# JNP-Solutions/Slacken

Hardware: AMD Instinct MI355X
Metric: classify_throughput_150bp_standard224scale (higher is better)
Workload: dtype u64

## Files before the change

slacken_amd/csrc/lane.hip:

```cpp
#include "engine.h"

#include <algorithm>
#include <cstddef>
#include <cstdio>
#include <cstdlib>

namespace slk {

#ifndef SLK_LANE_LW
#define SLK_LANE_LW 4
#endif
constexpr int LW = SLK_LANE_LW;
constexpr int QCAP = 128;
#ifndef SLK_SBLK
#define SLK_SBLK 5
#endif
constexpr int SBLK = SLK_SBLK;
#ifndef SLK_OMAP
#define SLK_OMAP 12
#endif
constexpr int OMAP = SLK_OMAP;
constexpr int OMAP_CNT_BITS = 10;
constexpr uint32_t OMAP_CNT_MASK = (1u << OMAP_CNT_BITS) - 1;

struct __attribute__((aligned(16))) LaneLds {
  uint64_t q_key[QCAP];
  uint32_t q_meta[QCAP];
  uint64_t stash[128];
  uint32_t found[64];
  uint4 sbuf[(SBLK - 1) * 64];
  uint32_t omap[OMAP * 64];
  uint32_t o_flags[64];
  uint64_t rb[64];
  uint16_t q_ord[QCAP];
};

#ifdef SLK_TUNING
#define SLK_TUNE(...) __VA_ARGS__
#define SLK_TUNE_ON(bit) ((dbg & (bit)) != 0)
#else
#define SLK_TUNE(...)
#define SLK_TUNE_ON(bit) false
#endif

#ifndef SLK_PROBE_NT
#define SLK_PROBE_NT 0
#endif
__device__ __forceinline__ ulonglong2 SLK_PROBE_LOAD(const ulonglong2 *p) {
#if SLK_PROBE_NT
  ulonglong2 v;
  v.x = __builtin_nontemporal_load(&p->x);
  v.y = __builtin_nontemporal_load(&p->y);
  return v;
#else
  return *p;
#endif
}

__device__ __forceinline__ void lane_wave_sync() {
  __builtin_amdgcn_fence(__ATOMIC_RELEASE, "wavefront");
  __builtin_amdgcn_wave_barrier();
  __builtin_amdgcn_fence(__ATOMIC_ACQUIRE, "wavefront");
}
__device__ __forceinline__ uint64_t lmin64(uint64_t a, uint64_t b) { return a < b ? a : b; }

template <bool LONG>
__device__ __forceinline__ void fold_hit(LaneLds *L, uint32_t *ocnt, bool in, uint32_t meta, int32_t taxon) {
  if (in && taxon != 0) {
    const int owner = meta & 63;
    const int32_t kmers = (int32_t)((meta >> 7) & 0x1FFF);
    if (meta & 64) atomicAdd(&L->o_flags[owner], 1u);
    uint32_t slot = (uint32_t)(((uint64_t)((uint32_t)taxon * 0x9E3779B1u) * (uint32_t)OMAP) >> 32);
    int p = 0;
    if (LONG) {
      for (; p < OMAP; p++) {
        uint32_t old = atomicCAS(&L->omap[slot * 64 + owner], 0u, (uint32_t)taxon);
        if (old == 0u || old == (uint32_t)taxon) { atomicAdd(&ocnt[slot * 64 + owner], (uint32_t)kmers); break; }
        slot = (slot + 1 == (uint32_t)OMAP) ? 0u : slot + 1;
      }
    } else {
      const uint32_t fresh = ((uint32_t)taxon << OMAP_CNT_BITS) | (uint32_t)kmers;
      for (; p < OMAP; p++) {
        uint32_t old = atomicCAS(&L->omap[slot * 64 + owner], 0u, fresh);
        if (old == 0u) break;
        if ((old >> OMAP_CNT_BITS) == (uint32_t)taxon) { atomicAdd(&L->omap[slot * 64 + owner], (uint32_t)kmers); break; }
        slot = (slot + 1 == (uint32_t)OMAP) ? 0u : slot + 1;
      }
    }
    if (p == OMAP) atomicOr(&L->o_flags[owner], 0x80000000u);
  }
}

constexpr int PG = 64 / LPB;
template <bool HITS, bool LONG>
__device__ __forceinline__ int probe_batch(LaneLds *L, uint32_t *ocnt, const TableView &T, int qhead, int qn, int cnt, int lane, int dbg,
                                           int32_t *hit_meta, int32_t *hit_taxon) {
  const uint64_t NO_TAG = ~0ULL;
  const bool in = lane < cnt;
  const int qi = (qhead + lane) & (QCAP - 1);
  const uint64_t key = L->q_key[qi];
  const uint32_t meta = L->q_meta[qi];
  const uint32_t ord = HITS ? L->q_ord[qi] : 0u;
  const uint64_t h = fmix64(key);
  uint32_t home;
  uint64_t rem_hi;
  table_slot(T.g, h, home, rem_hi);
  uint4 st;
  const uint32_t disp = (meta >> 20) & 255;
  st.x = table_bucket(T.g, home, disp);
  st.y = 0;
  const uint64_t tag = in ? (rem_hi + disp) : NO_TAG;
  st.z = (uint32_t)tag; st.w = (uint32_t)(tag >> 32);
  ((uint4 *)L->stash)[lane] = st;
  L->found[lane] = 0;
  lane_wave_sync();
  const int g = lane / LPB, c = lane % LPB;
  const uint64_t tmask = (1ULL << T.g.taxon_bits) - 1;
  const char *cellbase = (const char *)T.cells + c * 16;
  ulonglong2 cell[LPB];
#pragma unroll
  for (int s = 0; s < LPB; s++) {
    uint32_t bkt = ((const uint4 *)L->stash)[s * PG + g].x;
    SLK_TUNE(if (dbg & 4) bkt &= 1023u;)
    cell[s] = SLK_PROBE_LOAD((const ulonglong2 *)(cellbase + ((uint64_t)bkt << BUCKET_SHIFT)));
  }
  constexpr uint64_t GROUP_LSB = LPB == 4 ? 0x1111111111111111ULL : 0x0101010101010101ULL;
  int requeued = 0;
#pragma unroll
  for (int s = 0; s < LPB; s++) {
    const uint2 tg = *(const uint2 *)&((const uint4 *)L->stash)[s * PG + g].z;
    const uint64_t want = ((uint64_t)tg.y << 32) | tg.x;
    const bool act = want != NO_TAG;
    const bool e0 = cell[s].x == 0, e1 = cell[s].y == 0;
    const bool m0 = act && !e0 && cell_tag(T.g, cell[s].x) == want;
    const bool m1 = act && !e1 && cell_tag(T.g, cell[s].y) == want;
    if (m0 || m1) L->found[s * PG + g] = (uint32_t)((m0 ? cell[s].x : cell[s].y) & tmask);
    const bool closed = T.g.flag != 0 && c == 0 && (cell[s].x & T.g.flag) == 0;
    const uint64_t B = __ballot(m0 || m1 || e0 || e1 || !act || closed);
    uint64_t any = B;
#pragma unroll
    for (int i = 1; i < LPB; i <<= 1) any |= any >> i;
    if ((any & GROUP_LSB) != GROUP_LSB) {
      const int qj = (qhead + s * PG + g) & (QCAP - 1);
      const uint32_t m_old = L->q_meta[qj];
      const bool again = c == 0 && ((B >> (g * LPB)) & ((1u << LPB) - 1)) == 0 && (int)((m_old >> 20) & 255) < T.max_disp;
      const uint64_t k_old = L->q_key[qj];
      const uint16_t o_old = HITS ? L->q_ord[qj] : (uint16_t)0;
      const uint64_t R = __ballot(again);
      lane_wave_sync();
      if (again) {
        const int slot = (qhead + qn + requeued + __builtin_amdgcn_mbcnt_hi((uint32_t)(R >> 32), __builtin_amdgcn_mbcnt_lo((uint32_t)R, 0))) & (QCAP - 1);
        L->q_key[slot] = k_old;
        L->q_meta[slot] = m_old + (1u << 20);
        if (HITS) L->q_ord[slot] = o_old;
      }
      requeued += __popcll(R);
    }
  }
  lane_wave_sync();
  const int32_t taxon = (int32_t)L->found[lane];
  if (!SLK_TUNE_ON(2)) fold_hit<LONG>(L, ocnt, in, meta, taxon);
  if (HITS && in) {
    const uint64_t at = L->rb[meta & 63] + ord;
    hit_taxon[at] = ext_taxon(T, taxon);
    hit_meta[at] = pack_meta((int32_t)((meta >> 7) & 0x1FFF), 1, (meta >> 6) & 1);
  }
  lane_wave_sync();
  return requeued;
}

#ifndef SLK_STREAM_NT
#define SLK_STREAM_NT 0
#endif
#ifndef SLK_APPLY_ROWS
#define SLK_APPLY_ROWS 4
#endif
template <class T> __device__ __forceinline__ T SLK_STREAM_LOAD(const T *p) {
#if SLK_STREAM_NT
  return __builtin_nontemporal_load(p);
#else
  return *p;
#endif
}
template <class T> __device__ __forceinline__ void SLK_STREAM_STORE(T *p, T v) {
#if SLK_STREAM_NT
  __builtin_nontemporal_store(v, p);
#else
  *p = v;
#endif
}

__device__ __forceinline__ uint64_t lane_readlane64(uint64_t v, int src) {
  uint32_t lo = __builtin_amdgcn_readlane((uint32_t)v, src), hi = __builtin_amdgcn_readlane((uint32_t)(v >> 32), src);
  return ((uint64_t)hi << 32) | lo;
}
__device__ __forceinline__ uint32_t shard_owner(uint64_t key, uint32_t ns) {
  const uint64_t h = fmix64(key);
  return (ns & (ns - 1)) == 0 ? (uint32_t)(h & (ns - 1)) : (uint32_t)(h % ns);
}
__device__ __forceinline__ uint64_t side_load(const ShardIO &S, uint64_t batch, int lane) {
  const uint64_t i = batch * 64 + (uint64_t)lane;
  return i < S.side_n ? (uint64_t)SLK_STREAM_LOAD(&S.side_keys[i]) : 0;
}
__device__ __forceinline__ void side_probe(LaneLds *L, const TableView &T, const ShardIO &S, int lane, uint64_t batch, uint64_t key, int dbg) {
  const uint64_t base = batch * 64;
  if (base >= S.side_n) return;
  const uint64_t i = base + (uint64_t)lane;
  const bool in = i < S.side_n;
  const uint64_t h = fmix64(key);
  uint32_t home;
  uint64_t rem_hi;
  table_slot(T.g, h, home, rem_hi);
  const uint64_t tag = in ? rem_hi : ~0ULL;
  uint4 st;
  st.x = home; st.y = 0; st.z = (uint32_t)tag; st.w = (uint32_t)(tag >> 32);
  ((uint4 *)L->stash)[lane] = st;
  L->found[lane] = 0;
  lane_wave_sync();
  const int g = lane / LPB, c = lane % LPB;
  const uint64_t tmask = (1ULL << T.g.taxon_bits) - 1;
  const char *cellbase = (const char *)T.cells + c * 16;
  ulonglong2 cell[LPB];
#pragma unroll
  for (int s = 0; s < LPB; s++) {
    uint32_t bkt = ((const uint4 *)L->stash)[s * PG + g].x;
    SLK_TUNE(if (dbg & 4) bkt &= 1023u;)
    cell[s] = SLK_PROBE_LOAD((const ulonglong2 *)(cellbase + ((uint64_t)bkt << BUCKET_SHIFT)));
  }
  uint32_t unresolved = 0;
#pragma unroll
  for (int s = 0; s < LPB; s++) {
    const uint2 tg = *(const uint2 *)&((const uint4 *)L->stash)[s * PG + g].z;
    const uint64_t want = ((uint64_t)tg.y << 32) | tg.x;
    const bool act = want != ~0ULL;
    const bool e0 = cell[s].x == 0, e1 = cell[s].y == 0;
    const bool m0 = act && !e0 && cell_tag(T.g, cell[s].x) == want;
    const bool m1 = act && !e1 && cell_tag(T.g, cell[s].y) == want;
    if (m0 || m1) L->found[s * PG + g] = (uint32_t)((m0 ? cell[s].x : cell[s].y) & tmask);
    const bool closed = T.g.flag != 0 && c == 0 && (cell[s].x & T.g.flag) == 0;
    const uint64_t B = __ballot(m0 || m1 || e0 || e1 || !act || closed);
    if (((B >> (g * LPB)) & ((1u << LPB) - 1)) == 0) unresolved |= 1u << s;
  }
  lane_wave_sync();
  int32_t taxon = (int32_t)L->found[lane];
  const uint32_t ur = (uint32_t)__shfl((int)unresolved, (lane % PG) * LPB);
  if (in && ((ur >> (lane / PG)) & 1)) {
    for (int d = 1; d <= T.max_disp; d++) {
      const ulonglong2 *b = (const ulonglong2 *)(T.cells + ((uint64_t)table_bucket(T.g, home, (uint32_t)d) * CELLS));
      const uint64_t want = rem_hi | (uint64_t)d;
      bool has_empty = false, closed = false;
      int32_t hit = 0;
#pragma unroll
      for (int q = 0; q < LPB; q++) {
        const ulonglong2 v = b[q];
        has_empty |= (v.x == 0) | (v.y == 0);
        if (q == 0) closed = T.g.flag != 0 && (v.x & T.g.flag) == 0;
        if (v.x != 0 && cell_tag(T.g, v.x) == want) hit = (int32_t)(v.x & tmask);
        if (v.y != 0 && cell_tag(T.g, v.y) == want) hit = (int32_t)(v.y & tmask);
      }
      if (hit) { taxon = hit; break; }
      if (has_empty || closed) break;
    }
  }
  if (in && !SLK_TUNE_ON(128)) SLK_STREAM_STORE(&S.side_out[i], ext_taxon(T, taxon));
  lane_wave_sync();
}

template <bool HITS>
__device__ __forceinline__ void apply_rows(LaneLds *L, const ApplyJob &J, int lane, uint64_t row0, uint32_t nrows) {
  const uint32_t ns = (uint32_t)J.n_shards;
  constexpr int U = SLK_APPLY_ROWS;
  for (uint32_t b = 0; b < nrows; b += U) {
    uint64_t at[U];
    bool in[U];
#pragma unroll
    for (int u = 0; u < U; u++) {
      in[u] = false;
      at[u] = 0;
      if (b + u < nrows) {
        uint32_t off = 0;
        for (uint32_t sh = 0; sh < ns; sh++) {
          const uint4 e = J.batch_log[(row0 + b + u) * ns + sh];
          const uint32_t cnt = e.z;
          if (cnt == 0) continue;
          if ((uint32_t)lane >= off && (uint32_t)lane < off + cnt) {
            in[u] = true;
            const uint32_t i = (uint32_t)lane - off;
            at[u] = (uint64_t)sh * J.cap + (i < e.w ? e.x + i : e.y + (i - e.w));
          }
          off += cnt;
        }
      }
    }
    uint32_t meta[U];
    int32_t taxon[U];
#pragma unroll
    for (int u = 0; u < U; u++) {
      meta[u] = in[u] ? SLK_STREAM_LOAD(&J.send_meta[at[u]]) : 0u;
      taxon[u] = in[u] ? SLK_STREAM_LOAD(&J.taxa[at[u]]) : 0;
    }
#pragma unroll
    for (int u = 0; u < U; u++) {
      if (b + u < nrows) {
        int32_t t = taxon[u];
        if (in[u]) {
          if (HITS) {
            const uint64_t hat = L->rb[meta[u] & 63] + (meta[u] >> 20);
            J.A.span_taxon[hat] = t;
            J.A.span_meta[hat] = pack_meta((int32_t)((meta[u] >> 7) & 0x1FFF), 1, (meta[u] >> 6) & 1);
          }
          if (J.to_dense != nullptr && t > 0) t = t < J.n_to_dense ? J.to_dense[t] : 0;
        }
        fold_hit<false>(L, nullptr, in[u], meta[u], t);
      }
    }
    lane_wave_sync();
  }
}

template <bool HITS>
__device__ __forceinline__ void emit_batch(LaneLds *L, const FusedArgs &A, const ShardIO &S, const ApplyJob &J, int qhead, int cnt, int lane,
                                           uint64_t row, uint64_t tile, uint32_t &ch_pos, uint32_t &ch_end, uint32_t &side_j, uint64_t &side_key, int dbg) {
  SLK_TUNE(if (dbg & 256) return;)
  const bool in = lane < cnt;
  const int qi = (qhead + lane) & (QCAP - 1);
  const uint64_t key = L->q_key[qi];
  const uint32_t meta = L->q_meta[qi] | (HITS ? (uint32_t)L->q_ord[qi] << 20 : 0u);
  const uint32_t ns = (uint32_t)S.n_shards;
  const uint32_t g = ns == 1 ? 0u : shard_owner(key, ns);
  uint32_t mycount = 0, rank = 0;
  for (uint32_t sh = 0; sh < ns; sh++) {
    const uint64_t m = __ballot(in && g == sh);
    if ((uint32_t)lane == sh) mycount = (uint32_t)__popcll(m);
    if (g == sh) rank = __builtin_amdgcn_mbcnt_hi((uint32_t)(m >> 32), __builtin_amdgcn_mbcnt_lo((uint32_t)m, 0));
  }
  const uint32_t pos = ch_pos, room = ch_end - ch_pos;
  const bool need = (uint32_t)lane < ns && mycount > room;
  unsigned long long got = 0;
  if (need) got = atomicAdd(&S.cursors[lane], (unsigned long long)S.chunk);
  if (side_j < S.side_per_tile) {
    const uint64_t batch = tile * S.side_per_tile + side_j;
    const uint64_t k_now = side_key;
    side_j++;
    if (side_j < S.side_per_tile) side_key = side_load(S, batch + 1, lane);
    side_probe(L, A.T, S, lane, batch, k_now, dbg);
  }
  uint32_t fresh = 0xFFFFFFFFu;
  if (need) {
    if (got + S.chunk <= S.cap) fresh = (uint32_t)got;
    else atomicOr(A.status, 2);
  }
  if ((uint32_t)lane < ns) {
    S.batch_log[row * ns + (uint32_t)lane] = make_uint4(pos, fresh, mycount, room);
    if (need) { ch_pos = fresh == 0xFFFFFFFFu ? 0u : fresh + (mycount - room); ch_end = fresh == 0xFFFFFFFFu ? 0u : fresh + S.chunk; }
    else ch_pos = pos + mycount;
  }
  const uint32_t gpos = (uint32_t)__shfl((int)pos, (int)g), groom = (uint32_t)__shfl((int)room, (int)g), gfresh = (uint32_t)__shfl((int)fresh, (int)g);
  if (in) {
    const bool tail = rank >= groom;
    if ((!tail || gfresh != 0xFFFFFFFFu) && !SLK_TUNE_ON(32)) {
      const uint64_t at = (uint64_t)g * S.cap + (tail ? gfresh + (rank - groom) : gpos + rank);
      SLK_STREAM_STORE(&S.send_keys[at], (int64_t)key);
      SLK_STREAM_STORE(&S.send_meta[at], meta);
    }
  }
  lane_wave_sync();
}

__device__ __forceinline__ uint4 lane_node(const uint4 *nodes, int32_t ntax, int32_t t) {
  return ((uint32_t)t < (uint32_t)ntax) ? nodes[t] : make_uint4(0u, 0x40000000u + (uint32_t)t, 0x40000000u + (uint32_t)t, 0u);
}
__device__ __forceinline__ int lane_code(uint32_t c) {
  const uint32_t VM = (1u << 1) | (1u << 3) | (1u << 7) | (1u << 20) | (1u << 21);
  bool ok = ((c & 0xC0) == 0x40) && ((VM >> (c & 31)) & 1);
  uint32_t t = (c >> 1) & 3;
  t ^= t >> 1;
  return ok ? (int)t : 5;
}

__device__ __forceinline__ uint4 stream_refill(LaneLds *L, int lane, const uint8_t *seq, uint32_t p, uint32_t n, uint32_t room) {
  uint4 v[SBLK];
#pragma unroll
  for (int i = 0; i < SBLK; i++) {
    v[i] = make_uint4(0, 0, 0, 0);
    if (p + 16u * i < n) v[i] = load_block16(seq + p + 16u * i, room - (p + 16u * i));
  }
#pragma unroll
  for (int i = 1; i < SBLK; i++) L->sbuf[(i - 1) * 64 + lane] = v[i];
  return v[0];
}

#ifndef SLK_PACKED_STREAM
#define SLK_PACKED_STREAM 1
#endif
#ifndef SLK_PACK_ROUNDS
#define SLK_PACK_ROUNDS 2
#endif
constexpr uint32_t PACK_MAX_SPAN = 10880;
constexpr uint32_t PACK_WORDS = PACK_MAX_SPAN / 16 + 1;
constexpr int PACK_LOADS = (PACK_MAX_SPAN + 1023) / 1024;
static_assert((size_t)PACK_WORDS * 6 <= (size_t)(SBLK - 1) * 64 * 16, "the packed tile lives in the lane-wise stream's LDS slots");
__device__ __forceinline__ void pack16(const uint4 v, uint32_t &codes, uint32_t &valid) {
  const uint32_t VM = (1u << 1) | (1u << 3) | (1u << 7) | (1u << 20) | (1u << 21);
  const uint32_t w[4] = {v.x, v.y, v.z, v.w};
  codes = 0; valid = 0;
#pragma unroll
  for (int d = 0; d < 4; d++) {
    uint32_t t = (w[d] >> 1) & 0x03030303u;
    t ^= (t >> 1) & 0x01010101u;
    t = (t | (t >> 6) | (t >> 12) | (t >> 18)) & 0xFFu;
    codes |= t << (8 * d);
#pragma unroll
    for (int b = 0; b < 4; b++) {
      const uint32_t c = (w[d] >> (8 * b)) & 0xFFu;
      const uint32_t ok = (((c & 0xC0u) == 0x40u) ? 1u : 0u) & (VM >> (c & 31u));
      valid |= (ok & 1u) << (4 * d + b);
    }
  }
}
__device__ __forceinline__ uint2 packed_take(const uint32_t *pcodes, const uint16_t *pvalid, uint32_t s) {
  const uint32_t wi = s >> 4, bo = s & 15u;
  const uint64_t c64 = (uint64_t)pcodes[wi] | ((uint64_t)pcodes[wi + 1] << 32);
  const uint32_t v32 = (uint32_t)pvalid[wi] | ((uint32_t)pvalid[wi + 1] << 16);
  return make_uint2((uint32_t)(c64 >> (2 * bo)), (v32 >> bo) & 0xFFFFu);
}

#ifndef SLK_LANE_WPS
#define SLK_LANE_WPS 0
#endif
#if SLK_LANE_WPS > 0
#define LANE_BOUNDS __launch_bounds__(LW * 64, SLK_LANE_WPS)
#else
#define LANE_BOUNDS __launch_bounds__(LW * 64) __attribute__((amdgpu_waves_per_eu(4)))
#endif

__device__ __forceinline__ int route_by_length(uint64_t len, uint32_t long_max, uint32_t b0, uint32_t b1, uint32_t b2, uint32_t seg_min_len,
                                               uint32_t wave_min, uint32_t wave_ratio_q10) {
  if (long_max != 0 && len <= long_max) return (len > b0) + (len > b1) + (len > b2);
  if (seg_min_len != 0 && len >= seg_min_len) return HandOn::SEG;
  int c = HandOn::WAVE_CLASSES - 1;
  for (uint64_t b = ((uint64_t)wave_min * wave_ratio_q10) >> 10; c > 0 && len >= b; b = (b * wave_ratio_q10) >> 10) c--;
  return HandOn::WAVE0 + c;
}
__device__ __attribute__((noinline)) void hand_on(unsigned long long *hdr, uint32_t *lists, uint64_t stride, uint64_t long_cap, uint32_t long_max,
                                                  uint32_t b0, uint32_t b1, uint32_t b2, uint32_t seg_min_len, uint32_t wave_min,
                                                  uint32_t wave_ratio_q10, const uint64_t *offsets, const uint64_t *mate_offsets, bool dfr,
                                                  bool too_long, uint64_t r, int lane, bool from_long) {
  const uint64_t DM = __ballot(dfr);
  int route = from_long ? HandOn::LATE : HandOn::REST;
  if (!from_long && dfr && too_long) {
    uint64_t len = offsets[r + 1] - offsets[r];
    if (mate_offsets) len += mate_offsets[r + 1] - mate_offsets[r];
    route = route_by_length(len, long_max, b0, b1, b2, seg_min_len, wave_min, wave_ratio_q10);
  }
  if (!from_long && lane == 0) atomicAdd(&hdr[HandOn::HANDED], (unsigned long long)__popcll(DM));
  for (int l = from_long ? HandOn::LATE : 0; l <= HandOn::LATE; l++) {
    const uint64_t M = __ballot(dfr && route == l);
    if (M == 0) continue;
    const int leader = __ffsll((long long)M) - 1;
    unsigned long long at = 0;
    if (lane == leader) at = atomicAdd(&hdr[HandOn::count_word(l)], (unsigned long long)__popcll(M));
    at = lane_readlane64(at, leader);
    if (dfr && route == l)
      lists[HandOn::list_at(l, stride, long_cap) + at + __builtin_amdgcn_mbcnt_hi((uint32_t)(M >> 32), __builtin_amdgcn_mbcnt_lo((uint32_t)M, 0))] = (uint32_t)r;
  }
}

__global__ void __launch_bounds__(256) route_kernel(FusedArgs A) {
  constexpr int PER = 8, NL = HandOn::LISTS;
  __shared__ uint32_t cnt[NL];
  __shared__ unsigned long long base[NL];
  const uint64_t chunk = 256 * PER, chunks = (A.R + chunk - 1) / chunk;
  for (uint64_t c = blockIdx.x; c < chunks; c += gridDim.x) {
    if (threadIdx.x < NL) cnt[threadIdx.x] = 0;
    __syncthreads();
    int route[PER];
    uint32_t rank[PER];
#pragma unroll
    for (int j = 0; j < PER; j++) {
      const uint64_t r = c * chunk + (uint64_t)j * 256 + threadIdx.x;
      route[j] = -1;
      rank[j] = 0;
      if (r < A.R) {
        uint64_t len = A.offsets[r + 1] - A.offsets[r];
        if (A.mate_offsets) len += A.mate_offsets[r + 1] - A.mate_offsets[r];
        route[j] = len <= 1000 ? (int)HandOn::SHORT : route_by_length(len, A.long_max, A.long_bound[0], A.long_bound[1], A.long_bound[2],
                                                                      A.seg_min_len, A.wave_min, A.wave_ratio_q10);
        rank[j] = atomicAdd(&cnt[route[j]], 1u);
      }
    }
    __syncthreads();
    if (threadIdx.x < NL && cnt[threadIdx.x] != 0)
      base[threadIdx.x] = atomicAdd(&A.hand_hdr[HandOn::count_word((int)threadIdx.x)], (unsigned long long)cnt[threadIdx.x]);
    if (threadIdx.x == 0) {
      uint32_t handed = 0;
      for (int l = 0; l < NL; l++) if (l != HandOn::SHORT) handed += cnt[l];
      if (handed) atomicAdd(&A.hand_hdr[HandOn::HANDED], (unsigned long long)handed);
    }
    __syncthreads();
#pragma unroll
    for (int j = 0; j < PER; j++)
      if (route[j] >= 0)
        A.hand_lists[HandOn::list_at(route[j], A.hand_stride, A.hand_long_cap) + base[route[j]] + rank[j]] =
            (uint32_t)(c * chunk + (uint64_t)j * 256 + threadIdx.x);
    __syncthreads();
  }
}
void launch_route(const FusedArgs &A, hipStream_t s) {
  if (A.R == 0) return;
  hipLaunchKernelGGL(route_kernel, dim3((unsigned)std::min<uint64_t>((A.R + 2047) / 2048, 2048)), dim3(256), 0, s, A);
}

template <bool HITS, bool LONG>
__device__ __forceinline__ void resolve_lane(LaneLds *L, uint32_t *ocnt, const FusedArgs &A, int lane, uint64_t r, uint32_t oflags, int32_t total,
                                             int32_t nhits, int32_t np, int dbg) {
  const int32_t nd = (int32_t)oflags;
  uint32_t *const ecnt = LONG ? ocnt : L->omap;
  int D = 0;
  for (int s = 0; s < OMAP; s++) {
    const uint32_t e = L->omap[s * 64 + lane];
    if (e != 0) {
      if (LONG) ocnt[D * 64 + lane] = ocnt[s * 64 + lane];
      L->omap[D * 64 + lane] = e;
      D++;
    }
  }
#define ENT_TAXON(j) (LONG ? (int32_t)L->omap[(j) * 64 + lane] : (int32_t)(L->omap[(j) * 64 + lane] >> OMAP_CNT_BITS))
#define ENT_COUNT(j) (LONG ? (int32_t)ecnt[(j) * 64 + lane] : (int32_t)(ecnt[(j) * 64 + lane] & OMAP_CNT_MASK))
  int32_t maxTaxon = D ? ENT_TAXON(0) : 0;
  const int32_t c0 = D ? ENT_COUNT(0) : 0;
  uint32_t *const tin = (uint32_t *)L, *const tout = tin + OMAP * 64;
  static_assert(offsetof(LaneLds, omap) >= 2 * OMAP * 64 * sizeof(uint32_t), "the intervals alias the queue and the read stream's slots");
  uint32_t m_in = 0, m_out = 0;
  int32_t sum_all = c0;
  if (D >= 2 && !SLK_TUNE_ON(16)) {
#pragma unroll
    for (int j = 0; j < OMAP; j++) {
      if (j < D) {
        const uint4 nj = lane_node(A.nodes, A.ntax, ENT_TAXON(j));
        tin[j * 64 + lane] = nj.y;
        tout[j * 64 + lane] = nj.z;
      }
    }
    maxTaxon = 0;
    sum_all = 0;
    int32_t best = 0;
    for (int a = 0; a < D; a++) {
      const uint32_t ain = tin[a * 64 + lane], aout = tout[a * 64 + lane];
      int32_t score = 0;
      for (int b = 0; b < D; b++)
        score += (tin[b * 64 + lane] <= ain && ain <= tout[b * 64 + lane]) ? ENT_COUNT(b) : 0;
      sum_all += ENT_COUNT(a);
      if (score > best) {
        maxTaxon = ENT_TAXON(a); best = score; m_in = ain; m_out = aout;
      } else if (score == best) {
        if (m_in <= ain && ain <= m_out) {
        } else if (ain <= m_in && m_in <= aout) {
          maxTaxon = ENT_TAXON(a); m_in = ain; m_out = aout;
        } else {
          int32_t x = (int32_t)lane_node(A.nodes, A.ntax, maxTaxon).x;
          uint4 nx = make_uint4(0, 0, 0, 0);
          while (x != 0) {
            nx = lane_node(A.nodes, A.ntax, x);
            if (nx.y <= ain && ain <= nx.z) break;
            x = (int32_t)nx.x;
          }
          if (x == 0) { x = 1; nx = lane_node(A.nodes, A.ntax, 1); }
          maxTaxon = x; m_in = nx.y; m_out = nx.z;
        }
      }
    }
  }
  for (int32_t c = 0; c < A.C; c++) {
    const double required = ceil(__dmul_rn(A.thr.v[c], (double)total));
    int32_t mt = maxTaxon;
    if (D < 2 || SLK_TUNE_ON(16)) {
      if ((double)c0 < required) mt = 0;
    } else {
      uint32_t cin = m_in, cout = m_out;
      uint4 cur = make_uint4(0, 0, 0, 0);
      bool have_cur = false;
      while (mt != 0) {
        int32_t ms = 0;
        bool side = false;
        int up = -1;
        uint32_t up_in = 0;
        for (int j = 0; j < D; j++) {
          const uint32_t jin = tin[j * 64 + lane], jout = tout[j * 64 + lane];
          const bool inside = cin <= jin && jin <= cout;
          ms += inside ? ENT_COUNT(j) : 0;
          const bool above = !inside && jin <= cin && cin <= jout;
          side = side || (!inside && !above);
          if (above && (up < 0 || jin > up_in)) { up = j; up_in = jin; }
        }
        if ((double)ms >= required) break;
        if (ms == sum_all) { mt = 0; break; }
        if (!side) {
          mt = ENT_TAXON(up); cin = up_in; cout = tout[up * 64 + lane];
          have_cur = false;
        } else {
          if (!have_cur) cur = lane_node(A.nodes, A.ntax, mt);
          mt = (int32_t)cur.x;
          if (mt != 0) { cur = lane_node(A.nodes, A.ntax, mt); have_cur = true; cin = cur.y; cout = cur.z; }
        }
      }
    }
    bool classified = (mt != 0) && (nd >= A.min_hit_groups);
    A.out_taxon[(uint64_t)c * A.out_stride + r] = classified ? ext_taxon(A.T, mt) : 0;
    A.out_classified[(uint64_t)c * A.out_stride + r] = classified ? 1 : 0;
  }
#undef ENT_TAXON
#undef ENT_COUNT
  if (A.out_nd) A.out_nd[r] = nd;
  if (A.out_tk) A.out_tk[r] = total;
  if (A.out_nh) A.out_nh[r] = nhits;
  if (HITS) A.span_count[r] = nhits;
  if (A.out_np) A.out_np[r] = np;
}

template <bool W5, int MODE, bool HITS, bool LONG>
__device__ __forceinline__ void lane_body(const FusedArgs &A, const ShardIO &S, const ApplyJob *Jp, int32_t *defer, uint32_t max_len, int dbg) {
  extern __shared__ __attribute__((aligned(16))) unsigned char lds_raw[];
  const int lane = threadIdx.x & 63;
  const int wib = __builtin_amdgcn_readfirstlane(threadIdx.x >> 6);
  const ScanParams P = A.P;
  const int k = P.k, m = P.m, w = P.w;
  const size_t fixed = HITS ? sizeof(LaneLds) : offsetof(LaneLds, rb);
  const size_t win_bytes = W5 ? 0 : (size_t)w * 64 * sizeof(uint64_t);
  const size_t per_wave = fixed + win_bytes + (LONG ? (size_t)OMAP * 64 * sizeof(uint32_t) : 0);
  LaneLds *L = (LaneLds *)(lds_raw + (size_t)wib * per_wave);
  uint64_t *win = (uint64_t *)((unsigned char *)L + fixed);
  uint32_t *ocnt = LONG ? (uint32_t *)((unsigned char *)L + fixed + win_bytes) : nullptr;
  const bool paired = A.mate_bases != nullptr;
  const bool scans = MODE != LANE_EMIT || A.R != 0;
  const uint64_t bases_end = scans ? A.offsets[A.R] : 0, mates_end = (scans && paired) ? A.mate_offsets[A.R] : 0;
  uint64_t cls_n[5] = {0, 0, 0, 0, 0}, cls_tiles[5] = {0, 0, 0, 0, 0};
  uint64_t ntiles = (A.R + 63) / 64;
  if (LONG) {
    ntiles = 0;
#pragma unroll
    for (int c = 0; c < 5; c++) {
      cls_n[c] = c == 0 ? (A.route_first ? A.hand_hdr[HandOn::N_SHORT] : 0ULL) : A.hand_hdr[c - 1];
      cls_tiles[c] = (cls_n[c] + 63) / 64;
      ntiles += cls_tiles[c];
    }
  }
  const uint64_t nwaves = (uint64_t)gridDim.x * LW;
  const uint64_t etiles = ntiles;
  const uint64_t atiles = MODE == LANE_EMIT ? (Jp->A.R + 63) / 64 : 0;
  if (MODE == LANE_EMIT) ntiles = max(etiles, atiles);
  uint32_t ch_pos = 0, ch_end = 0;

  for (uint64_t tile = (uint64_t)blockIdx.x * LW + wib, it = 0;; it++) {
    if (LONG) {
      if (it) {
        unsigned long long t = 0;
        if (lane == 0) t = atomicAdd(&A.hand_hdr[HandOn::LONG_DRAW], 1ULL);
        tile = nwaves + lane_readlane64(t, 0);
      }
    } else if (MODE == LANE_EMIT) {
      if (it) {
        unsigned long long t = 0;
        if (lane == 0) t = atomicAdd(&S.cursors[S.n_shards], 1ULL);
        tile = nwaves + lane_readlane64(t, 0);
      }
    } else if (it) {
      tile += nwaves;
    }
    if (tile >= ntiles) break;
    uint64_t unit = tile * 64 + lane;
    bool have = unit < A.R;
    uint64_t r = unit;
    if (LONG) {
      uint64_t local = tile;
      int c = 4;
#pragma unroll
      for (int i = 4; i > 0; i--) if (c == i && local >= cls_tiles[i]) { local -= cls_tiles[i]; c = i - 1; }
      unit = local * 64 + lane;
      have = unit < cls_n[c];
      const uint32_t *const cl = A.hand_lists + HandOn::list_at(c == 0 ? (int)HandOn::SHORT : c - 1, A.hand_stride, A.hand_long_cap);
      r = have ? (uint64_t)cl[unit] : 0;
    }
    const uint8_t *seq = A.bases;
    uint32_t n = 0, n2 = 0;
    uint32_t room = 0;
    if (have) {
      uint64_t o = A.offsets[r];
      seq = A.bases + o;
      n = (uint32_t)(A.offsets[r + 1] - o);
      room = clamp_room(bases_end - o);
      SLK_TUNE(if (dbg & 8) { seq = A.bases + A.offsets[r & 1023]; room = clamp_room(bases_end - A.offsets[r & 1023]); })
      if (paired) n2 = (uint32_t)(A.mate_offsets[r + 1] - A.mate_offsets[r]);
    }
    bool too_long = have && ((uint64_t)n + n2 > max_len);
    bool fin = !have || too_long;
    uint64_t row = 0, row0 = 0;
    if (MODE == LANE_EMIT && tile < etiles) row = row0 = (span_region(A.offsets, A.mate_offsets, tile * 64) >> 6) + tile;
    const uint64_t rbase = (HITS && have) ? span_region(A.offsets, A.mate_offsets, r) : 0;
    if (HITS && MODE != LANE_EMIT) L->rb[lane] = rbase;
#pragma unroll
    for (int s = 0; s < OMAP; s++) L->omap[s * 64 + lane] = 0;
    if (LONG) {
#pragma unroll
      for (int s = 0; s < OMAP; s++) ocnt[s * 64 + lane] = 0;
    }
    L->o_flags[lane] = 0;
    if (MODE == LANE_EMIT && tile < atiles) {
      const uint64_t r2 = tile * 64 + lane;
      const bool have2 = r2 < Jp->A.R;
      const uint2 tr = Jp->tile_rows[tile];
      if (HITS) L->rb[lane] = have2 ? span_region(Jp->A.offsets, Jp->A.mate_offsets, r2) : 0;
      lane_wave_sync();
      apply_rows<HITS>(L, *Jp, lane, tr.x, tr.y);
      const bool dfr2 = have2 && (Jp->defer[r2] != 0 || (L->o_flags[lane] & 0x80000000u));
      const uint64_t DM = __ballot(dfr2);
      if (DM != 0 && lane == 0) atomicAdd(Jp->n_deferred, (unsigned long long)__popcll(DM));
      if (have2) {
        if (dfr2) {
          Jp->defer[r2] = 1;
          if (Jp->A.out_nh) Jp->A.out_nh[r2] = 0;
          if (HITS) Jp->A.span_count[r2] = 0;
        } else {
          const int2 ri = Jp->read_info[r2];
          resolve_lane<HITS, false>(L, nullptr, Jp->A, lane, r2, L->o_flags[lane], ri.x, ri.y, 0, dbg);
        }
      }
      lane_wave_sync();
    }
    uint32_t pos = 0;
    int mate = 0;
    uint32_t cur = 0, b1 = 0, b2 = 0, b3 = 0;
    int sb = 1;
    bool packed = false;
    uint32_t s0 = 0;
    uint32_t *const pcodes = (uint32_t *)L->sbuf;
    uint16_t *const pvalid = (uint16_t *)(pcodes + PACK_WORDS);
    constexpr bool CAN_PACK = SLK_PACKED_STREAM && !LONG && MODE == LANE_LOCAL;
    if (CAN_PACK && !paired) {
      const uint64_t t0 = tile * 64, t1 = min(A.R, t0 + 64);
      const uint64_t span_o = A.offsets[t0], span = A.offsets[t1] - span_o;
      if (span <= PACK_MAX_SPAN && __ballot(!fin) != 0) {
        packed = true;
        s0 = have ? (uint32_t)(A.offsets[r] - span_o) : 0;
        const uint8_t *tb = A.bases + span_o;
        const uint32_t troom = clamp_room(bases_end - span_o), sp = (uint32_t)span;
        constexpr int PG0 = (PACK_LOADS + SLK_PACK_ROUNDS - 1) / SLK_PACK_ROUNDS;
#pragma unroll
        for (int j0 = 0; j0 < PACK_LOADS; j0 += PG0) {
          uint4 v[PG0];
#pragma unroll
          for (int j = 0; j < PG0; j++) {
            const uint32_t cb = (uint32_t)(j0 + j) * 1024u + (uint32_t)lane * 16u;
            v[j] = make_uint4(0, 0, 0, 0);
            if (j0 + j < PACK_LOADS && cb < sp) v[j] = load_block16(tb + cb, troom - cb);
          }
#pragma unroll
          for (int j = 0; j < PG0; j++) {
            const uint32_t cb = (uint32_t)(j0 + j) * 1024u + (uint32_t)lane * 16u;
            if (j0 + j < PACK_LOADS && cb < sp + 16u) {
              uint32_t cw, vw;
              pack16(v[j], cw, vw);
              pcodes[cb >> 4] = cw;
              pvalid[cb >> 4] = (uint16_t)vw;
            }
          }
        }
        lane_wave_sync();
      }
    }
    if (!fin && n > 0) {
      if (CAN_PACK && packed) {
        const uint2 pk = packed_take(pcodes, pvalid, s0);
        cur = pk.x; b1 = pk.y;
      } else {
        uint4 v = stream_refill(L, lane, seq, 0, n, room);
        cur = v.x; b1 = v.y; b2 = v.z; b3 = v.w;
      }
    }
    int run_class = 0;
    uint32_t run_len = 0, nvalid = 0;
    uint64_t fwd = 0, rc = 0;
    uint64_t k1 = ~0ULL, p1 = ~0ULL, p2 = ~0ULL, m41 = ~0ULL;
    uint64_t pre = ~0ULL;
    uint64_t cur_val = 0;
    int32_t cur_run = 0;
    bool first = true, have_last = false;
    uint64_t last_key = 0;
    int32_t total = 0, np = 0, nhits = 0;
    uint32_t side_j = (MODE == LANE_EMIT && S.side_n != 0 && tile < etiles) ? 0u : 0xFFFFFFFFu;
    uint64_t side_key = (MODE == LANE_EMIT && S.side_n != 0 && S.side_per_tile != 0 && tile < etiles) ? side_load(S, tile * S.side_per_tile, lane) : 0;
    int qn = 0;
    int qhead = 0;
    int tphase = 0;

    const uint32_t VM = (1u << 1) | (1u << 3) | (1u << 7) | (1u << 20) | (1u << 21);
    while (__ballot(!fin) != 0) {
      if (!W5 && tphase == 0) pre = ~0ULL;
      const bool act = !fin;
      const bool is_end = pos >= n;
      bool okc;
      uint32_t t;
      if (CAN_PACK && packed) {
        t = cur & 3u;
        okc = (b1 & 1u) != 0;
      } else {
        const uint32_t c = cur & 0xFF;
        okc = ((c & 0xC0) == 0x40) && ((VM >> (c & 31)) & 1);
        t = (c >> 1) & 3;
        t ^= t >> 1;
      }
      const int cls = is_end ? -1 : (okc ? 1 : 0);
      const bool run_end = act && run_len > 0 && cls != run_class;
      const bool seqrun = run_class == 1 && nvalid >= (uint32_t)k;
      const bool seq_close = run_end && seqrun;
      const bool amb_close = run_end && !seqrun && run_len >= (uint32_t)k;
      const int32_t ord0 = nhits;
      total += amb_close ? (int32_t)run_len - (k - 1) : 0;
      if (HITS && amb_close) {
        A.span_meta[rbase + ord0] = pack_meta((int32_t)run_len - (k - 1), 2, 0);
        A.span_taxon[rbase + ord0] = -1;
      }
      nhits += amb_close ? 1 : 0;
      first = first && !amb_close;
      const uint64_t ekey = cur_val;
      const int32_t ekmers = cur_run;
      run_len = run_end ? 0u : run_len;
      const bool proc = act && !is_end;
      const bool new_run = proc && run_len == 0;
      run_class = new_run ? cls : run_class;
      nvalid = new_run ? 0u : nvalid;
      cur_run = (new_run || seq_close) ? 0 : cur_run;
      run_len += proc ? 1u : 0u;
      const bool nt = proc && okc;
      nvalid += nt ? 1u : 0u;
      fwd = (fwd << 2) | ((uint64_t)t << P.sh);
      rc = ((rc >> 2) | ((uint64_t)(3 - t) << 62)) & P.keep;
      const bool havekey = nt && nvalid >= (uint32_t)m;
      const uint64_t canon = (P.canonical && rc < fwd) ? rc : fwd;
      const uint64_t key = (canon ^ P.xmask) & P.smask;
      uint64_t minv;
      if (W5) {
        const uint64_t p = lmin64(key, k1);
        const uint64_t m4 = lmin64(p, p2);
        minv = lmin64(key, m41);
        k1 = key; p2 = p1; p1 = p; m41 = m4;
      } else {
        const uint64_t kk = havekey ? key : ~0ULL;
        pre = lmin64(pre, kk);
        minv = (tphase == w - 1) ? pre : lmin64(pre, win[(tphase + 1) * 64 + lane]);
        win[tphase * 64 + lane] = kk;
      }
      const bool havewin = havekey && nvalid >= (uint32_t)k;
      const bool start = havewin && cur_run == 0;
      const bool same = havewin && cur_run != 0 && minv == cur_val;
      const bool change = havewin && cur_run != 0 && minv != cur_val;
      const bool emit = seq_close || change;
      cur_val = (start || change) ? minv : cur_val;
      cur_run = (start || change) ? 1 : (same ? cur_run + 1 : cur_run);
      pos += proc ? 1u : 0u;
      const bool refill = proc && (pos & 15) == 0;
      if (CAN_PACK && packed) {
        cur = proc ? (cur >> 2) : cur;
        b1 = proc ? (b1 >> 1) : b1;
        if (__ballot(refill) != 0) {
          if (refill && pos < n) {
            const uint2 pk = packed_take(pcodes, pvalid, s0 + pos);
            cur = pk.x; b1 = pk.y;
          }
        }
      } else {
        const bool nextdw = proc && (pos & 3) == 0;
        cur = nextdw ? b1 : (proc ? (cur >> 8) : cur);
        b1 = nextdw ? b2 : b1;
        b2 = nextdw ? b3 : b2;
        if (__ballot(refill) != 0) {
          if (refill) {
            if (pos < n) {
              uint4 v;
              if (sb < SBLK) { v = L->sbuf[(sb - 1) * 64 + lane]; sb++; }
              else { v = stream_refill(L, lane, seq, pos, n, room); sb = 1; }
              cur = v.x; b1 = v.y; b2 = v.z; b3 = v.w;
            }
          }
        }
      }
      const bool at_end = act && is_end;
      if (__ballot(at_end) != 0) {
        if (at_end) {
          if (mate == 0 && paired) {
            if (HITS) {
              const int32_t ordb = ord0 + ((amb_close || emit) ? 1 : 0);
              A.span_meta[rbase + ordb] = pack_meta(-(k - 1), 3, 0);
              A.span_taxon[rbase + ordb] = -2;
            }
            nhits++;
            first = false;
            mate = 1;
            const uint64_t o2 = A.mate_offsets[r];
            seq = A.mate_bases + o2; n = (uint32_t)(A.mate_offsets[r + 1] - o2); room = clamp_room(mates_end - o2); pos = 0;
            if (n > 0) {
              uint4 v = stream_refill(L, lane, seq, 0, n, room);
              sb = 1;
              cur = v.x; b1 = v.y; b2 = v.z; b3 = v.w;
            }
          } else {
            fin = true;
          }
        }
      }
      if (!W5) {
        if (tphase == w - 1) {
          uint64_t sm = ~0ULL;
          for (int j = w - 1; j >= 0; j--) { sm = lmin64(sm, win[j * 64 + lane]); win[j * 64 + lane] = sm; }
          tphase = 0;
        } else {
          tphase++;
        }
      }
      const bool distinct = emit && (first || !(have_last && ekey == last_key));
      last_key = emit ? ekey : last_key;
      have_last = have_last || emit;
      first = first && !emit;
      total += emit ? ekmers : 0;
      np += emit ? 1 : 0;
      nhits += emit ? 1 : 0;
      uint64_t E = __ballot(emit);
      if (E != 0) {
        if (emit) {
          int slot = (qhead + qn + __builtin_amdgcn_mbcnt_hi((uint32_t)(E >> 32), __builtin_amdgcn_mbcnt_lo((uint32_t)E, 0))) & (QCAP - 1);
          L->q_key[slot] = ekey;
          if (HITS) L->q_ord[slot] = (uint16_t)ord0;
          L->q_meta[slot] = (uint32_t)lane | (distinct ? 64u : 0u) | ((uint32_t)ekmers << 7);
        }
        qn += __popcll(E);
        while (qn >= 64) {
          lane_wave_sync();
          int back = 0;
          if (MODE == LANE_EMIT) emit_batch<HITS>(L, A, S, *Jp, qhead, 64, lane, row++, tile, ch_pos, ch_end, side_j, side_key, dbg);
          else if (!SLK_TUNE_ON(1)) back = probe_batch<HITS, LONG>(L, ocnt, A.T, qhead, qn, 64, lane, dbg, A.span_meta, A.span_taxon);
          qhead = (qhead + 64) & (QCAP - 1);
          qn += back - 64;
        }
      }
    }
    while (qn > 0) {
      lane_wave_sync();
      const int cnt = min(qn, 64);
      int back = 0;
      if (MODE == LANE_EMIT) emit_batch<HITS>(L, A, S, *Jp, qhead, cnt, lane, row++, tile, ch_pos, ch_end, side_j, side_key, dbg);
      else if (!SLK_TUNE_ON(1)) back = probe_batch<HITS, LONG>(L, ocnt, A.T, qhead, qn, cnt, lane, dbg, A.span_meta, A.span_taxon);
      qhead = (qhead + cnt) & (QCAP - 1);
      qn += back - cnt;
    }
    lane_wave_sync();
    if (MODE == LANE_EMIT) {
      if (tile < etiles) {
        if (have) S.read_info[r] = make_int2(total, nhits);
        if (lane == 0) S.tile_rows[tile] = make_uint2((uint32_t)row0, (uint32_t)(row - row0));
      }
      while (side_j < S.side_per_tile) {
        const uint64_t batch = tile * S.side_per_tile + side_j;
        const uint64_t k_now = side_key;
        side_j++;
        if (side_j < S.side_per_tile) side_key = side_load(S, batch + 1, lane);
        side_probe(L, A.T, S, lane, batch, k_now, dbg);
      }
    }

    if (MODE == LANE_LOCAL) {
      const uint32_t oflags = have ? L->o_flags[lane] : 0u;
      const bool dfr = have && (too_long || (oflags & 0x80000000u));
      if (__ballot(dfr) != 0)
        hand_on(A.hand_hdr, A.hand_lists, A.hand_stride, A.hand_long_cap, A.long_max, A.long_bound[0], A.long_bound[1], A.long_bound[2],
                A.seg_min_len, A.wave_min, A.wave_ratio_q10, A.offsets, A.mate_offsets, dfr, too_long, r, lane, LONG);
      if (have && !dfr) resolve_lane<HITS, LONG>(L, ocnt, A, lane, r, oflags, total, nhits, np, dbg);
    } else {
      if (have && too_long) defer[r] = 1;
    }
    lane_wave_sync();
  }
  if (MODE == LANE_EMIT) {
    for (uint32_t sh = 0; sh < (uint32_t)S.n_shards; sh++) {
      const uint32_t p0 = __builtin_amdgcn_readlane(ch_pos, sh), p1 = __builtin_amdgcn_readlane(ch_end, sh);
      for (uint32_t i = p0 + (uint32_t)lane; i < p1; i += 64) S.send_keys[(uint64_t)sh * S.cap + i] = 0;
    }
  }
}

template <bool W5, int MODE, bool HITS, bool LONG>
__global__ void LANE_BOUNDS lane_kernel(FusedArgs A, ShardIO S, int32_t *defer, uint32_t max_len, int dbg) {
  lane_body<W5, MODE, HITS, LONG>(A, S, nullptr, defer, max_len, dbg);
}
template <bool W5, bool HITS>
__global__ void LANE_BOUNDS lane_step_kernel(FusedArgs A, ShardIO S, ApplyJob J, int32_t *defer, uint32_t max_len, int dbg) {
  lane_body<W5, LANE_EMIT, HITS, false>(A, S, &J, defer, max_len, dbg);
}

static size_t lane_lds_per_wave(bool hits, bool w5, int w, bool lng) {
  return (hits ? sizeof(LaneLds) : offsetof(LaneLds, rb)) + (w5 ? 0 : (size_t)w * 64 * sizeof(uint64_t)) + (lng ? (size_t)OMAP * 64 * sizeof(uint32_t) : 0);
}

template <bool HITS, bool LONG>
static void launch_lane_mode(const FusedArgs &A, int32_t *defer, uint32_t max_len, hipStream_t s) {
  if (A.R == 0) return;
  const bool w5 = A.P.w == 5;
  const size_t per_wave = lane_lds_per_wave(HITS, w5, A.P.w, LONG);
  static const int extra_lds = getenv("SLK_LANE_EXTRA_LDS") ? atoi(getenv("SLK_LANE_EXTRA_LDS")) : 0;
  size_t lds = per_wave * LW + (size_t)extra_lds;
  uint64_t tiles = (A.R + 63) / 64;
  uint64_t blocks = (tiles + LW - 1) / LW;
  static const int bpc = getenv("SLK_LANE_BLOCKS_PER_CU") ? atoi(getenv("SLK_LANE_BLOCKS_PER_CU")) : 0;
  if (bpc > 0 && blocks > (uint64_t)256 * bpc) blocks = (uint64_t)256 * bpc;
  if (LONG && blocks > 256 * 5) blocks = 256 * 5;
  dim3 g((unsigned)blocks), b(LW * 64);
#ifdef SLK_TUNING
  static const int dbg = getenv("SLK_DEBUG_ABLATE") ? atoi(getenv("SLK_DEBUG_ABLATE")) : 0;
#else
  const int dbg = 0;
#endif
  static bool occ_printed = false;
  if (getenv("SLK_DEBUG_OCC") && !occ_printed) {
    occ_printed = true;
    int nb = 0;
    (void)hipOccupancyMaxActiveBlocksPerMultiprocessor(&nb, w5 ? (const void *)lane_kernel<true, LANE_LOCAL, HITS, LONG> : (const void *)lane_kernel<false, LANE_LOCAL, HITS, LONG>, LW * 64, lds);
    fprintf(stderr, "[slk] lane kernel: %zu B LDS per block, %d blocks (%d waves) resident per CU\n", lds, nb, nb * LW);
  }
  if (w5) hipLaunchKernelGGL((lane_kernel<true, LANE_LOCAL, HITS, LONG>), g, b, lds, s, A, ShardIO{}, defer, max_len, dbg);
  else hipLaunchKernelGGL((lane_kernel<false, LANE_LOCAL, HITS, LONG>), g, b, lds, s, A, ShardIO{}, defer, max_len, dbg);
}

void launch_lane(const FusedArgs &A, int32_t *defer, uint32_t max_len, hipStream_t s) {
  if (A.span_taxon) launch_lane_mode<true, false>(A, defer, max_len, s);
  else launch_lane_mode<false, false>(A, defer, max_len, s);
}
void launch_lane_long(const FusedArgs &A, uint32_t max_len, hipStream_t s) {
  if (A.span_taxon) launch_lane_mode<true, true>(A, nullptr, max_len, s);
  else launch_lane_mode<false, true>(A, nullptr, max_len, s);
}

template <bool W5, bool HITS>
static void launch_step_mode(const FusedArgs &A, const ShardIO &S, const ApplyJob &J, int32_t *defer, uint32_t max_len, hipStream_t s) {
  const uint64_t tiles = std::max((A.R + 63) / 64, (J.A.R + 63) / 64);
  if (tiles == 0) return;
  const size_t lds = lane_lds_per_wave(HITS, W5, A.P.w, false) * LW;
  static int resident[2][2] = {{0, 0}, {0, 0}};
  static int cus = 0;
  if (cus == 0) {
    int dev = 0;
    (void)hipGetDevice(&dev);
    if (hipDeviceGetAttribute(&cus, hipDeviceAttributeMultiprocessorCount, dev) != hipSuccess || cus <= 0) cus = 256;
  }
  int nb = W5 ? resident[1][HITS] : 0;
  if (nb == 0) {
    if (hipOccupancyMaxActiveBlocksPerMultiprocessor(&nb, (const void *)lane_step_kernel<W5, HITS>, LW * 64, lds) != hipSuccess || nb <= 0) nb = 4;
    if (W5) resident[1][HITS] = nb;
  }
  static const int bpc = getenv("SLK_STEP_BLOCKS_PER_CU") ? atoi(getenv("SLK_STEP_BLOCKS_PER_CU")) : 0;
  if (bpc > 0) nb = bpc;
  const uint64_t blocks = std::min<uint64_t>((tiles + LW - 1) / LW, (uint64_t)cus * nb);
#ifdef SLK_TUNING
  static const int dbg = getenv("SLK_DEBUG_ABLATE") ? atoi(getenv("SLK_DEBUG_ABLATE")) : 0;
#else
  const int dbg = 0;
#endif
  hipLaunchKernelGGL((lane_step_kernel<W5, HITS>), dim3((unsigned)blocks), dim3(LW * 64), lds, s, A, S, J, defer, max_len, dbg);
}
void launch_lane_step(const FusedArgs &A, const ShardIO &S, const ApplyJob &J, int32_t *defer, uint32_t max_len, hipStream_t s) {
  const bool hits = A.R ? A.span_taxon != nullptr : J.A.span_taxon != nullptr;
  if (A.P.w == 5) { if (hits) launch_step_mode<true, true>(A, S, J, defer, max_len, s); else launch_step_mode<true, false>(A, S, J, defer, max_len, s); }
  else { if (hits) launch_step_mode<false, true>(A, S, J, defer, max_len, s); else launch_step_mode<false, false>(A, S, J, defer, max_len, s); }
}

}
```

Before: 1136.

## Stage batch log in LDS and double-buffer apply gathers against folds

apply_rows now loads a chunk of the batch log cooperatively into LDS (sbuf), one coalesced load per lane, instead of every lane reading each log entry from global memory. It then software-pipelines two groups of rows so the send_meta/taxa gathers for the next group are in flight while the current group is folded, with the rows-per-group default lowered from 4 to 2. The defer flag and read_info loads are hoisted ahead of apply_rows so their latency overlaps it. In exchange the code uses more registers, reuses sbuf (so it assumes sbuf is free at this point), and gathers unconditionally at index 0 for inactive lanes.

```diff
diff --git a/slacken_amd/csrc/lane.hip b/slacken_amd/csrc/lane.hip
--- a/slacken_amd/csrc/lane.hip
+++ b/slacken_amd/csrc/lane.hip
@@ -173,7 +173,7 @@
 #define SLK_STREAM_NT 0
 #endif
 #ifndef SLK_APPLY_ROWS
-#define SLK_APPLY_ROWS 4
+#define SLK_APPLY_ROWS 2
 #endif
 template <class T> __device__ __forceinline__ T SLK_STREAM_LOAD(const T *p) {
 #if SLK_STREAM_NT
@@ -266,53 +266,84 @@
   lane_wave_sync();
 }
 
+constexpr int APPLY_LOG = (SBLK - 1) * 64;
+static_assert(APPLY_LOG >= 64, "a pass holds at least one row of the log at 64 owners");
+struct ApplyGroup {
+  uint32_t in;
+  uint32_t meta[SLK_APPLY_ROWS];
+  int32_t taxon[SLK_APPLY_ROWS];
+};
+__device__ __forceinline__ void apply_issue(const ApplyJob &J, const uint4 *lg, int lane, uint32_t ns, uint32_t r0, uint32_t nr, ApplyGroup &G) {
+  constexpr int U = SLK_APPLY_ROWS;
+  uint64_t at[U];
+  G.in = 0;
+#pragma unroll
+  for (int u = 0; u < U; u++) {
+    at[u] = 0;
+    if (r0 + u < nr) {
+      uint32_t off = 0;
+      for (uint32_t sh = 0; sh < ns; sh++) {
+        const uint4 e = lg[(r0 + u) * ns + sh];
+        const uint32_t cnt = (uint32_t)__builtin_amdgcn_readfirstlane((int)e.z);
+        if (cnt == 0) continue;
+        if ((uint32_t)lane >= off && (uint32_t)lane < off + cnt) {
+          G.in |= 1u << u;
+          const uint32_t i = (uint32_t)lane - off;
+          at[u] = (uint64_t)sh * J.cap + (i < e.w ? e.x + i : e.y + (i - e.w));
+        }
+        off += cnt;
+      }
+    }
+  }
+#pragma unroll
+  for (int u = 0; u < U; u++) {
+    G.meta[u] = SLK_STREAM_LOAD(&J.send_meta[at[u]]);
+    G.taxon[u] = SLK_STREAM_LOAD(&J.taxa[at[u]]);
+  }
+}
+template <bool HITS>
+__device__ __forceinline__ void apply_fold(LaneLds *L, const ApplyJob &J, uint32_t r0, uint32_t nr, const ApplyGroup &G) {
+  constexpr int U = SLK_APPLY_ROWS;
+#pragma unroll
+  for (int u = 0; u < U; u++) {
+    if (r0 + u < nr) {
+      const bool in = (G.in >> u) & 1;
+      int32_t t = in ? G.taxon[u] : 0;
+      if (in) {
+        if (HITS) {
+          const uint64_t hat = L->rb[G.meta[u] & 63] + (G.meta[u] >> 20);
+          J.A.span_taxon[hat] = t;
+          J.A.span_meta[hat] = pack_meta((int32_t)((G.meta[u] >> 7) & 0x1FFF), 1, (G.meta[u] >> 6) & 1);
+        }
+        if (J.to_dense != nullptr && t > 0) t = t < J.n_to_dense ? J.to_dense[t] : 0;
+      }
+      fold_hit<false>(L, nullptr, in, G.meta[u], t);
+    }
+  }
+}
 template <bool HITS>
 __device__ __forceinline__ void apply_rows(LaneLds *L, const ApplyJob &J, int lane, uint64_t row0, uint32_t nrows) {
   const uint32_t ns = (uint32_t)J.n_shards;
-  constexpr int U = SLK_APPLY_ROWS;
-  for (uint32_t b = 0; b < nrows; b += U) {
-    uint64_t at[U];
-    bool in[U];
-#pragma unroll
-    for (int u = 0; u < U; u++) {
-      in[u] = false;
-      at[u] = 0;
-      if (b + u < nrows) {
-        uint32_t off = 0;
-        for (uint32_t sh = 0; sh < ns; sh++) {
-          const uint4 e = J.batch_log[(row0 + b + u) * ns + sh];
-          const uint32_t cnt = e.z;
-          if (cnt == 0) continue;
-          if ((uint32_t)lane >= off && (uint32_t)lane < off + cnt) {
-            in[u] = true;
-            const uint32_t i = (uint32_t)lane - off;
-            at[u] = (uint64_t)sh * J.cap + (i < e.w ? e.x + i : e.y + (i - e.w));
-          }
-          off += cnt;
-        }
-      }
-    }
-    uint32_t meta[U];
-    int32_t taxon[U];
-#pragma unroll
-    for (int u = 0; u < U; u++) {
-      meta[u] = in[u] ? SLK_STREAM_LOAD(&J.send_meta[at[u]]) : 0u;
-      taxon[u] = in[u] ? SLK_STREAM_LOAD(&J.taxa[at[u]]) : 0;
-    }
-#pragma unroll
-    for (int u = 0; u < U; u++) {
-      if (b + u < nrows) {
-        int32_t t = taxon[u];
-        if (in[u]) {
-          if (HITS) {
-            const uint64_t hat = L->rb[meta[u] & 63] + (meta[u] >> 20);
-            J.A.span_taxon[hat] = t;
-            J.A.span_meta[hat] = pack_meta((int32_t)((meta[u] >> 7) & 0x1FFF), 1, (meta[u] >> 6) & 1);
-          }
-          if (J.to_dense != nullptr && t > 0) t = t < J.n_to_dense ? J.to_dense[t] : 0;
-        }
-        fold_hit<false>(L, nullptr, in[u], meta[u], t);
-      }
+  constexpr uint32_t U = SLK_APPLY_ROWS;
+  const uint32_t per_pass = (uint32_t)APPLY_LOG / ns;
+  uint4 *const lg = (uint4 *)L->sbuf;
+  for (uint32_t p0 = 0; p0 < nrows; p0 += per_pass) {
+    const uint32_t nr = min(per_pass, nrows - p0), ne = nr * ns;
+    const uint4 *const src = J.batch_log + (row0 + p0) * ns;
+    uint4 v[APPLY_LOG / 64];
+#pragma unroll
+    for (int j = 0; j < APPLY_LOG / 64; j++)
+      v[j] = src[min((uint32_t)(j * 64 + lane), ne - 1)];
+#pragma unroll
+    for (int j = 0; j < APPLY_LOG / 64; j++) lg[j * 64 + lane] = v[j];
+    lane_wave_sync();
+    ApplyGroup Ga, Gb;
+    apply_issue(J, lg, lane, ns, 0, nr, Ga);
+    for (uint32_t g = 0; g < nr; g += 2 * U) {
+      apply_issue(J, lg, lane, ns, g + U, nr, Gb);
+      apply_fold<HITS>(L, J, g, nr, Ga);
+      apply_issue(J, lg, lane, ns, g + 2 * U, nr, Ga);
+      apply_fold<HITS>(L, J, g + U, nr, Gb);
     }
     lane_wave_sync();
   }
@@ -710,9 +741,11 @@
       const bool have2 = r2 < Jp->A.R;
       const uint2 tr = Jp->tile_rows[tile];
       if (HITS) L->rb[lane] = have2 ? span_region(Jp->A.offsets, Jp->A.mate_offsets, r2) : 0;
+      const int32_t dfr_emit = have2 ? Jp->defer[r2] : 0;
+      const int2 ri = have2 ? Jp->read_info[r2] : make_int2(0, 0);
       lane_wave_sync();
       apply_rows<HITS>(L, *Jp, lane, tr.x, tr.y);
-      const bool dfr2 = have2 && (Jp->defer[r2] != 0 || (L->o_flags[lane] & 0x80000000u));
+      const bool dfr2 = have2 && (dfr_emit != 0 || (L->o_flags[lane] & 0x80000000u));
       const uint64_t DM = __ballot(dfr2);
       if (DM != 0 && lane == 0) atomicAdd(Jp->n_deferred, (unsigned long long)__popcll(DM));
       if (have2) {
@@ -721,7 +754,6 @@
           if (Jp->A.out_nh) Jp->A.out_nh[r2] = 0;
           if (HITS) Jp->A.span_count[r2] = 0;
         } else {
-          const int2 ri = Jp->read_info[r2];
           resolve_lane<HITS, false>(L, nullptr, Jp->A, lane, r2, L->o_flags[lane], ri.x, ri.y, 0, dbg);
         }
       }
```

Result: no change. 1136 (-0.1%).
